# maxpit/human-pose-estimation

Hardware: AMD Instinct MI355X
Metric: images/sec (224x224, batch 256/GPU) (higher is better)
Workload: dtype f32; 1 GPU; batch=256/GPU 224x224x3 synthetic images, fp32 ResNet-50 v1 + 3-iter regressor + SMPL LBS at all 3 stages (configs[1] at batch 256; the BASELINE metric batch); global_batch=256, parallelism=dp1 (batch shard, replicated weights), regressor=synthetic 'survey' variant, input=float32 images resident in HBM

## Files before the change

human-pose-estimation_amd/csrc/bf16_rows.h:

```cpp
#pragma once
#include <hip/hip_runtime.h>

#include "hpe_internal.h"

#define BKE 64
#define RF 32

#define HPE_WAIT_VMCNT(n) __builtin_amdgcn_s_waitcnt(0x0F70 | ((n) & 15) | (((n) >> 4) << 14))
#define HPE_WAIT_LGKM0() __builtin_amdgcn_s_waitcnt(0xC07F)
```

human-pose-estimation_amd/csrc/conv_chain_f32.hip:

```cpp
#include <hip/hip_runtime.h>
#include <stdint.h>

#include "hpe_internal.h"

typedef float f32x16 __attribute__((ext_vector_type(16)));
typedef float f32x4 __attribute__((ext_vector_type(4)));
typedef const __attribute__((address_space(4))) float* cfloat_p;
typedef const __attribute__((address_space(4))) f32x4* cf32x4_p;

namespace {

__device__ __forceinline__ void dma16(const void* src, void* lds_dst) {
    __builtin_amdgcn_global_load_lds((const __attribute__((address_space(1))) void*)src, (__attribute__((address_space(3))) void*)lds_dst, 16, 0, 0);
}
__device__ __forceinline__ void dma16_nt(const void* src, void* lds_dst) {
    __builtin_amdgcn_global_load_lds((const __attribute__((address_space(1))) void*)src, (__attribute__((address_space(3))) void*)lds_dst, 16, 0, 2);
}
__device__ __forceinline__ void lds_barrier() { asm volatile("s_waitcnt lgkmcnt(0)\n\ts_barrier" ::: "memory"); }
__device__ __forceinline__ void wait_dma_leaving(int n, bool exact_counts) {
    if (!exact_counts) n = 0;
    switch (n) {
        case 4: asm volatile("s_waitcnt vmcnt(4)" ::: "memory"); break;
        case 8: asm volatile("s_waitcnt vmcnt(8)" ::: "memory"); break;
        default: asm volatile("s_waitcnt vmcnt(0)" ::: "memory"); break;
    }
}

template <int C, int CP>
__global__ __launch_bounds__(256, 2) void chain_expand_reduce_f32_kernel(ChainArgsF32 p) {
    constexpr int BM = 64, NC = 64, C4 = 4 * C;
    constexpr int KSA = C / 32, KSB = NC / 32, NCH = C4 / NC;
    constexpr int SLAB = BM * 128;
    constexpr int QBYTES = KSB * SLAB, QBUFS = 32768 / QBYTES;
    constexpr int WA_SLAB = NC * 128, WB_SLAB = CP * 128;
    constexpr int AT_OFF = 0, Q_OFF = KSA * SLAB, WA_OFF = Q_OFF + QBUFS * QBYTES, WB_OFF = WA_OFF + KSA * WA_SLAB;
    constexpr int LDS_BYTES = WB_OFF + KSB * WB_SLAB;
    constexpr int RI = KSB * 2, WIB = KSB * CP / 32, ST = NC / 16;
    static_assert(C == 64 && CP == 64, "stage 2 only: one 32-channel block per wave in both GEMMs");
    static_assert(QBUFS == 2 && NCH == 4 && LDS_BYTES <= 80 * 1024, "geometry");
    static_assert(RI == 4 && WIB == 4 && ST == 4, "the counted waits below know 0 / 4 / 8 only");

    __shared__ __attribute__((aligned(16))) unsigned char lds[LDS_BYTES];

// ... 48 lines not shown
#pragma unroll
        for (int s = 0; s < KSB; ++s) {
            const char* base = WBb + (c * NC + s * 32) * 4;
#pragma unroll
            for (int i = 0; i < CP / 32; ++i)
                dma16(base + (size_t)(32 * i) * p.ldw2a * 4 + off_wb, lds + WB_OFF + s * WB_SLAB + (wave + 4 * i) * 1024);
        }
    };

    const int wm = wave >> 1, wn = wave & 1;
    const int ar = wm * 32 + (lane & 31);
    const int a_off = ar * 128, a_x = (ar >> 1) & 7;
    const int wr = wn * 32 + (lane & 31);
    const int w_off = wr * 128, w_x = (wr >> 1) & 7;

    f32x16 accB;
#pragma unroll
    for (int e = 0; e < 16; ++e) accB[e] = 0.f;

    issue_at();
    issue_res(0);
    issue_wa(0);
    issue_wb(0);
    issue_res(1);

#pragma unroll
    for (int c = 0; c < NCH; ++c) {
        const int qb = c % QBUFS;
        wait_dma_leaving(c == 0 ? WIB + (QBUFS - 1) * RI : ST, full_tile);
        lds_barrier();
        if (c > 0) issue_wb(c);
        if (c > 0 && c - 1 + QBUFS < NCH) issue_res(c - 1 + QBUFS);

        f32x16 accA;
#pragma unroll
        for (int e = 0; e < 16; ++e) accA[e] = 0.f;
#pragma unroll
        for (int sa = 0; sa < KSA; ++sa)
#pragma unroll
            for (int g = 0; g < 4; ++g) {
                const int lc = 2 * g + hi;
                const f32x4 fa = *reinterpret_cast<const f32x4*>(lds + AT_OFF + sa * SLAB + a_off + ((lc ^ a_x) << 4));
                const f32x4 fw = *reinterpret_cast<const f32x4*>(lds + WA_OFF + sa * WA_SLAB + w_off + ((lc ^ w_x) << 4));
#pragma unroll
                for (int ks = 0; ks < 4; ++ks) accA = __builtin_amdgcn_mfma_f32_32x32x2f32(fw[ks], fa[ks], accA, 0, 0, 0);
            }

        {
            unsigned char* Qs = lds + Q_OFF + qb * QBYTES + wn * SLAB + a_off;
            cfloat_p scp = (cfloat_p)(p.scaleA + c * NC + wn * 32);
            cfloat_p shp = (cfloat_p)(p.shiftA + c * NC + wn * 32);
#pragma unroll
            for (int q = 0; q < 4; ++q) {
                unsigned char* qp = Qs + (((2 * q + hi) ^ a_x) << 4);
                const f32x4 rv = *reinterpret_cast<const f32x4*>(qp);
                const f32x4 sc_lo = *reinterpret_cast<cf32x4_p>(scp + 8 * q), sc_hi = *reinterpret_cast<cf32x4_p>(scp + 8 * q + 4);
                const f32x4 sh_lo = *reinterpret_cast<cf32x4_p>(shp + 8 * q), sh_hi = *reinterpret_cast<cf32x4_p>(shp + 8 * q + 4);
                f32x4 o;
#pragma unroll
                for (int k = 0; k < 4; ++k) {
                    const float sc = hi ? sc_hi[k] : sc_lo[k];
// ... 10 lines not shown
        {
            const unsigned char* Q = lds + Q_OFF + qb * QBYTES;
            constexpr int UPR = NC / 4;
#pragma unroll
            for (int pass = 0; pass < (BM * UPR) / 256; ++pass) {
                const int idx = pass * 256 + t;
                const int r = idx / UPR, u = idx - r * UPR;
                const f32x4 v = *reinterpret_cast<const f32x4*>(Q + (u >> 3) * SLAB + r * 128 + (((u & 7) ^ ((r >> 1) & 7)) << 4));
                const int m = m0 + r;
                if (m < p.M) __builtin_nontemporal_store(v, reinterpret_cast<f32x4*>(p.t3 + (size_t)m * C4 + c * NC + u * 4));
            }
        }
#pragma unroll
        for (int sb = 0; sb < KSB; ++sb) {
            const unsigned char* Q = lds + Q_OFF + qb * QBYTES + sb * SLAB;
#pragma unroll
            for (int g = 0; g < 4; ++g) {
                const int lc = 2 * g + hi;
                const f32x4 fa = *reinterpret_cast<const f32x4*>(Q + a_off + ((lc ^ a_x) << 4));
                const f32x4 fw = *reinterpret_cast<const f32x4*>(lds + WB_OFF + sb * WB_SLAB + w_off + ((lc ^ w_x) << 4));
#pragma unroll
                for (int ks = 0; ks < 4; ++ks) accB = __builtin_amdgcn_mfma_f32_32x32x2f32(fw[ks], fa[ks], accB, 0, 0, 0);
            }
        }
    }

    {
        unsigned char* Us = lds + AT_OFF + wn * SLAB + a_off;
        cfloat_p scp = (cfloat_p)(p.scaleB + wn * 32);
        cfloat_p shp = (cfloat_p)(p.shiftB + wn * 32);
#pragma unroll
        for (int q = 0; q < 4; ++q) {
            const f32x4 sc_lo = *reinterpret_cast<cf32x4_p>(scp + 8 * q), sc_hi = *reinterpret_cast<cf32x4_p>(scp + 8 * q + 4);
            const f32x4 sh_lo = *reinterpret_cast<cf32x4_p>(shp + 8 * q), sh_hi = *reinterpret_cast<cf32x4_p>(shp + 8 * q + 4);
            f32x4 o;
#pragma unroll
            for (int k = 0; k < 4; ++k) {
                const float sc = hi ? sc_hi[k] : sc_lo[k];
                const float sh = hi ? sh_hi[k] : sh_lo[k];
                o[k] = fmaxf(accB[4 * q + k] * sc + sh, 0.f);
            }
// ... 21 lines not shown
                else *reinterpret_cast<f32x4*>(p.u1 + (size_t)m * CP + u * 4) = v;
            }
        }
    }
}

}

bool hpe_chain_f32_supported(int C, int C4, int CP) { return C == 64 && C4 == 256 && CP == 64; }

hipError_t hpe_launch_chain_f32(const ChainArgsF32& p, int C, int C4, int CP, hipStream_t st) {
    if (!hpe_chain_f32_supported(C, C4, CP)) return hipErrorInvalidValue;
    if (p.M <= 0 || !p.t2 || !p.res || !p.w2c || !p.w2a || !p.t3 || !p.u1 || !p.scaleA || !p.shiftA || !p.scaleB || !p.shiftB) return hipErrorInvalidValue;
    if (p.ldw2c < C || p.ldw2a < C4 || (p.ldw2c % 4) != 0 || (p.ldw2a % 4) != 0) return hipErrorInvalidValue;
    if ((((uintptr_t)p.t2 | (uintptr_t)p.res | (uintptr_t)p.w2c | (uintptr_t)p.w2a | (uintptr_t)p.t3 | (uintptr_t)p.u1) & 15) != 0) return hipErrorInvalidValue;
    hipLaunchKernelGGL((chain_expand_reduce_f32_kernel<64, 64>), dim3((p.M + 63) / 64), dim3(256), 0, st, p);
    return hipGetLastError();
}

hipError_t hpe_chain_f32_occupancy(int* out) {
    return hipOccupancyMaxActiveBlocksPerMultiprocessor(out, reinterpret_cast<const void*>(chain_expand_reduce_f32_kernel<64, 64>), 256, 0);
}
```

human-pose-estimation_amd/csrc/conv_gemm.hip:

```cpp
#include <hip/hip_runtime.h>
#include <stdint.h>

#include "conv_gemm_common.h"
#include "gemm_contract.h"
#include "hpe_internal.h"

namespace {

template <int MODE, int BM, int BN, int WM, int WN>
__global__ __launch_bounds__(64 * WM * WN, (WM * WN) / 2) void conv_gemm_f32_dma_kernel(GemmArgs p) {
    constexpr int MT = BM / WM / 32;
    constexpr int NT = BN / WN / 32;
    constexpr int NW = WM * WN;
    constexpr int NTHR = 64 * NW;
    constexpr int AP = BM / (8 * NW);
    constexpr int BP = BN / (8 * NW);
    constexpr int EP = BN + 4;
    constexpr int BUF = (BM + BN) * BK;
    constexpr int LDS_FLOATS = (2 * BUF > BM * EP) ? 2 * BUF : BM * EP;
    static_assert(NW == 4 || NW == 8, "4 or 8 waves per workgroup");
    static_assert(AP >= 1 && BP >= 1, "tile too small for the wave count");

    __shared__ __attribute__((aligned(16))) float lds[LDS_FLOATS];

    const int total = p.n_mtiles * p.n_ntiles;
    const int bid = blockIdx.x;
    int tile, ks0 = 0, ks1 = p.K / BK, part = -1;
    if (p.split_k > 1) {
        tile = bid / p.split_k;
        part = bid - tile * p.split_k;
        const int S = p.K / BK;
        ks0 = (int)((long)part * S / p.split_k);
        ks1 = (int)((long)(part + 1) * S / p.split_k);
    } else {
        tile = xcd_remap(bid, total);
    }
// ... 36 lines not shown
#pragma unroll
    for (int j = 0; j < NT; ++j) {
        const int r = (wn * NT + j) * 32 + (lane & 31);
        b_row[j] = (BM + r) * BK;
        b_x[j] = (r >> 1) & 7;
    }
    const int hi = lane >> 5;

    f32x16 acc[MT][NT];
#pragma unroll
    for (int i = 0; i < MT; ++i)
#pragma unroll
        for (int j = 0; j < NT; ++j)
#pragma unroll
            for (int e = 0; e < 16; ++e) acc[i][j][e] = 0.f;

    constexpr int R_TPR = BN / 4, R_RPP = NTHR / R_TPR, R_NPASS = BM / R_RPP;
    constexpr bool R_PRE = (NW == 8) && R_NPASS <= 4;
    f32x4 rpre[R_PRE ? R_NPASS : 1];
    bool r_pre = false;
    if constexpr (R_PRE) {
        const int rr_ = t / R_TPR;
        const int n = n0 + (t - rr_ * R_TPR) * 4;
        r_pre = p.res != nullptr && p.res_prefetch && part < 0 && (n + 3) < p.N;
        if (r_pre) {
#pragma unroll
            for (int pass = 0; pass < R_NPASS; ++pass) {
                const int m = m0 + pass * R_RPP + rr_;
                rpre[pass] = HPE_RES_LOAD(reinterpret_cast<const f32x4*>(p.res + (size_t)(m < p.M ? m : p.M - 1) * p.ldres + n));
            }
        }
    }

    SlabPos sp = slab_seek<MODE>(p, ks0);

    auto issue_dma = [&](int slab, int buf) {
// ... 17 lines not shown
                                             (__attribute__((address_space(3))) void*)(lds + buf + (BM + (NW * i + wave) * 8) * BK), 16, 0,
                                             0);
        }
    };

    issue_dma(ks0, 0);
    __builtin_amdgcn_s_waitcnt(0x0F70);
    __syncthreads();

    for (int s = ks0; s < ks1; ++s) {
        const int cur = ((s - ks0) & 1) * BUF;
        if (s + 1 < ks1) {
            slab_advance<MODE>(p, sp);
            issue_dma(s + 1, BUF - cur);
        }
#pragma unroll
        for (int g = 0; g < 4; ++g) {
            f32x4 fa[MT], fb[NT];
            const int lc = 2 * g + hi;
#pragma unroll
            for (int i = 0; i < MT; ++i) fa[i] = *reinterpret_cast<const f32x4*>(&lds[cur + a_row[i] + ((lc ^ a_x[i]) << 2)]);
#pragma unroll
            for (int j = 0; j < NT; ++j) fb[j] = *reinterpret_cast<const f32x4*>(&lds[cur + b_row[j] + ((lc ^ b_x[j]) << 2)]);
#pragma unroll
            for (int ks = 0; ks < 4; ++ks)
#pragma unroll
                for (int i = 0; i < MT; ++i)
#pragma unroll
                    for (int j = 0; j < NT; ++j)
                        acc[i][j] = __builtin_amdgcn_mfma_f32_32x32x2f32(fa[i][ks], fb[j][ks], acc[i][j], 0, 0, 0);
        }
        __builtin_amdgcn_s_waitcnt(0x0F70);
        __syncthreads();
    }

    if (part >= 0) {
        f32x4* dst = reinterpret_cast<f32x4*>(p.partial) + (size_t)(tile * p.split_k + part) * (MT * NT * 4 * NTHR) + t;
#pragma unroll
        for (int i = 0; i < MT; ++i)
#pragma unroll
            for (int j = 0; j < NT; ++j)
#pragma unroll
                for (int qd = 0; qd < 4; ++qd) {
                    f32x4 v = {acc[i][j][4 * qd], acc[i][j][4 * qd + 1], acc[i][j][4 * qd + 2], acc[i][j][4 * qd + 3]};
                    dst[((i * NT + j) * 4 + qd) * NTHR] = v;
                }
        return;
    }
// ... 39 lines not shown
    }
    const f32x4 no_pre[1] = {{0.f, 0.f, 0.f, 0.f}};
    conv_epilogue<BM, BN, WM, WN>(p, lds, acc, mtile * BM, ntile * BN, t, lane, wm, wn, no_pre, false);
}

template <int MODE, int TILE>
hipError_t launch_cfg(GemmArgs& p, int splitk_min_slabs, hipStream_t st) {
    constexpr TileShape T = tile_shape(GEMM_K_F32, TILE);
    constexpr int BM = T.bm, BN = T.bn, WM = T.wm, WN = T.wn;
    p.n_mtiles = (p.M + BM - 1) / BM;
    p.n_ntiles = (p.N + BN - 1) / BN;
    const int grid = p.n_mtiles * p.n_ntiles;
    p.split_k = 1;
    if constexpr (WM * WN == 8) {
        p.res_prefetch = 1;
        hipLaunchKernelGGL((conv_gemm_f32_dma_kernel<MODE, BM, BN, WM, WN>), dim3(grid), dim3(512), 0, st, p);
        return hipGetLastError();
    } else {
        const int S = p.K / BK;
        if (p.partial && grid < 128 && S >= 2 * splitk_min_slabs) {
            int sk = 256 / grid;
            if (sk > S / splitk_min_slabs) sk = S / splitk_min_slabs;
            if (sk > 16) sk = 16;
            while (sk > 1 && (size_t)grid * sk * BM * BN > p.partial_floats) --sk;
            if (sk > 1) p.split_k = sk;
        }
        hipLaunchKernelGGL((conv_gemm_f32_dma_kernel<MODE, BM, BN, WM, WN>), dim3(grid * p.split_k), dim3(256), 0, st, p);
        hipError_t e = hipGetLastError();
        if (e != hipSuccess || p.split_k == 1) return e;
        hipLaunchKernelGGL((conv_gemm_fixup_kernel<BM, BN, WM, WN>), dim3(grid), dim3(256), 0, st, p);
        return hipGetLastError();
    }
}

template <int MODE>
hipError_t launch_mode(GemmArgs& p, int tile, int splitk_min_slabs, hipStream_t st) {
    switch (tile) {
        case TILE_128x128: return launch_cfg<MODE, TILE_128x128>(p, splitk_min_slabs, st);
        case TILE_128x64: return launch_cfg<MODE, TILE_128x64>(p, splitk_min_slabs, st);
        case TILE_64x64: return launch_cfg<MODE, TILE_64x64>(p, splitk_min_slabs, st);
        case TILE_64x128: return launch_cfg<MODE, TILE_64x128>(p, splitk_min_slabs, st);
        case TILE_128x128_W8: return launch_cfg<MODE, TILE_128x128_W8>(p, splitk_min_slabs, st);
// ... 24 lines not shown
```

human-pose-estimation_amd/csrc/conv_gemm_f32s.hip:

```cpp
#include <hip/hip_runtime.h>
#include <stdint.h>
#include <stdlib.h>

#include "conv_gemm_common.h"
#include "gemm_contract.h"
#include "hpe_internal.h"

namespace {

typedef __bf16 bf16x8 __attribute__((ext_vector_type(8)));

__device__ __forceinline__ void split3(const f32x4& lo, const f32x4& hi, bf16x8& h0, bf16x8& h1, bf16x8& h2) {
#pragma unroll
    for (int e = 0; e < 8; ++e) {
        const float x = e < 4 ? lo[e] : hi[e - 4];
        const __bf16 b0 = (__bf16)x;
        const float r1 = x - (float)b0;
        const __bf16 b1 = (__bf16)r1;
        const float r2 = r1 - (float)b1;
        h0[e] = b0;
        h1[e] = b1;
        h2[e] = (__bf16)r2;
    }
}

template <int MODE, int BM, int BN, int WM, int WN>
__global__ __launch_bounds__(64 * WM * WN, 2) void conv_gemm_f32s_dma_kernel(GemmArgs p) {
    constexpr int MT = BM / WM / 32;
    constexpr int NT = BN / WN / 32;
    constexpr int NW = WM * WN;
    constexpr int NTHR = 64 * NW;
    constexpr int AP = BM / (8 * NW);
    constexpr int BP = BN / (16 * NW);
    constexpr int A_BYTES = BM * BK * 4;
    constexpr int W_BYTES = BN * BK * 2;
    constexpr int BUF = A_BYTES + 3 * W_BYTES;
    constexpr int EPB = BM * (BN + 4) * 4;
    constexpr int LDS_BYTES = (2 * BUF > EPB) ? 2 * BUF : EPB;
    static_assert(NW == 4 || NW == 8, "4 or 8 waves per workgroup");
// ... 180 lines not shown
```

human-pose-estimation_amd/csrc/hpe_ctx.h:

```cpp
#pragma once
#include <hip/hip_runtime.h>

#include <cmath>
#include <cstdint>
#include <cstring>
#include <string>
#include <vector>

#include "../../include/hpe.h"
#include "hpe_internal.h"
#include "hpe_plan.h"

int fail(int code, const std::string& msg);

#define HIP_TRY(expr)                                                                                             \
    do {                                                                                                          \
        hipError_t _e = (expr);                                                                                   \
        if (_e != hipSuccess)                                                                                     \
            return fail(HPE_ERR_HIP, std::string(#expr) + ": " + hipGetErrorString(_e) + " (" __FILE__ ":" +      \
                                         std::to_string(__LINE__) + ")");                                         \
    } while (0)

struct ConvSpec {
    char name[24];
// ... 241 lines not shown
        if (_e != hipSuccess) return _e;         \
    } while (0)

enum { NEED_ENC = 1, NEED_REG = 2, NEED_SMPL = 4 };
int check_ready(hpe_ctx* c, int B, int need);

int finalize_impl(hpe_ctx* c);
void release_device_state(hpe_ctx* c);
int repack_encoder(hpe_ctx* c);

hipError_t run_conv(hpe_ctx* c, int idx, const ConvRoute& r, const float* x, int B, const float* res, int relu, float* y, hipStream_t st,
                    float* wino_v = nullptr, int slot = 0, const float* scale = nullptr, const float* shift = nullptr);
hipError_t run_conv_nhwc(hpe_ctx* c, int idx, const float* x, int B, const float* res, int relu, float* y, hipStream_t st,
                         const float* scale = nullptr, const float* shift = nullptr);
hipError_t run_chain(hpe_ctx* c, int i2c, bool first, const float* t2, const float* res, int B, float* t3, float* u1, hipStream_t st,
                     bool u1_slab8 = false);
hipError_t encoder_impl(hpe_ctx* c, const float* images, int B, float* features, int ldfeat, hipStream_t st);
hipError_t run_dense(hpe_ctx* c, const float* x, int lda, int M, int K, const float* w, int w_rows, int N, const float* scale, const float* shift,
                     const float* res, int ldres, int relu, float* y, int ldy, hipStream_t st, float* partial = nullptr, size_t partial_floats = 0);
hipError_t regress_impl(hpe_ctx* c, const float* th_prev, float* th_next, int B, hipStream_t st);
hipError_t features_proj(hpe_ctx* c, const float* features, int B, hipStream_t st);
hipError_t tail_impl(hpe_ctx* c, const float* feat, int B, const HpeOutputs* stage_outs, int n_outs, hipStream_t ts, hipEvent_t feat_free);
hipError_t join_tail(hpe_ctx* c, hipStream_t st);
int forward_impl(hpe_ctx* c, const float* images, int B, const HpeOutputs* stage_outs, int n_outs, hipStream_t st, bool pipelined);

size_t encoder_repack_reserve_floats();
int encoder_repack_reserve(hpe_ctx* c);
hipError_t encoder_repack_launch(hpe_ctx* c, const float* flat_dev, hipStream_t st);

hipError_t encoder_repack_stats_launch(hpe_ctx* c, hipStream_t st);

// ... 17 lines not shown
```

human-pose-estimation_amd/csrc/hpe_encoder.hip:

```cpp
#include <hip/hip_runtime.h>

#include <cmath>
#include <cstdint>
#include <cstdio>
#include <cstdlib>
#include <cstring>
#include <string>
#include <vector>

#include "hpe_ctx.h"

static hipError_t launch_gemm(hpe_ctx* c, GemmArgs& p, const ConvRoute& r, const void* w_split, hipStream_t st) {
    if (!r.concurrent) p.partial = c->partial, p.partial_floats = c->partial_floats;
    if (r.kernel == CONV_K_BF16 || r.kernel == CONV_K_BF16_P8) return hpe_launch_gemm_bf16(p, r.mode, r.tile, st);
    if (r.kernel != CONV_K_F32S) return hpe_launch_gemm(p, r.mode, r.tile, c->plan.splitk_min_slabs, st);
    if (!w_split) return hipErrorInvalidValue;
    p.w = static_cast<const float*>(w_split);
    p.w_piece = p.ldw;
    p.ldw *= 3;
    return hpe_launch_gemm_f32s(p, r.mode, r.tile, st);
}

hipError_t run_conv(hpe_ctx* c, int idx, const ConvRoute& r, const float* x, int B, const float* res, int relu, float* y, hipStream_t st,
                    float* wino_v, int slot, const float* scale, const float* shift) {
    const ConvSpec& s = specs()[idx];
    const ConvLayer& L = c->conv[idx];
    if (!scale) scale = L.scale;
    if (!shift) shift = L.shift;
    const int H = s.hin;
    const bool f2 = r.kernel == CONV_K_WINO || r.kernel == CONV_K_WINO_FUSED, f4 = r.kernel == CONV_K_WINO4 || r.kernel == CONV_K_WINO4_FUSED;
// ... 50 lines not shown

static hipError_t run_dual(hpe_ctx* c, int i2c, int i1, const ConvRoute& r, const float* t2, const float* x, int B, float* y, hipStream_t st) {
    const ConvSpec& s2 = specs()[i2c];
    const ConvSpec& s1 = specs()[i1];
    const ConvLayer& L = c->conv[i2c];
    GemmArgs p{};
    p.x = t2, p.x2 = x, p.w = L.w_dual, p.scale = c->ones, p.shift = L.shift_dual, p.y = y, p.zero = c->zeros;
    p.M = B * s2.hout * s2.hout, p.N = s2.cout, p.K = L.k_dual;
    p.k1_slabs = L.k1_dual / (c->bf16 ? 64 : 32), p.relu = 1;
    p.lda = s2.cin, p.ldw = L.k_dual, p.w_rows = round_up(s2.cout, 128), p.ldy = s2.cout;
    p.Hi = p.Wi = s1.hin, p.Cin = s1.cin, p.Ho = p.Wo = s1.hout, p.stride = s1.stride;
    return launch_gemm(c, p, r, L.w_dual_split, st);
}

hipError_t run_chain(hpe_ctx* c, int i2c, bool first, const float* t2, const float* res, int B, float* t3, float* u1, hipStream_t st,
                     bool u1_slab8) {
    const ConvSpec& s2 = specs()[i2c];
    const int inext = i2c + (first ? 2 : 1);
    const ConvSpec& sn = specs()[inext];
    const ConvLayer& L2 = c->conv[i2c];
    const ConvLayer& Ln = c->conv[inext];
    if (!c->bf16) {
        ChainArgsF32 q{};
        q.t2 = t2;
        q.res = res;
        q.w2c = L2.w;
        q.w2a = Ln.w;
        q.scaleA = L2.scale;
        q.shiftA = L2.shift;
        q.scaleB = Ln.scale;
        q.shiftB = Ln.shift;
        q.t3 = t3;
        q.u1 = u1;
        q.M = B * s2.hout * s2.hout;
        q.ldw2c = L2.k_pad;
        q.ldw2a = Ln.k_pad;
        q.u1_slab8 = u1_slab8 ? 1 : 0;
        return hpe_launch_chain_f32(q, s2.cin, s2.cout, sn.cout, st);
    }
    ChainArgs p{};
    p.t2 = reinterpret_cast<const __bf16*>(t2);
    if (first) {
        p.x2 = reinterpret_cast<const __bf16*>(res);
        p.w2c = reinterpret_cast<const __bf16*>(L2.w_dual);
        p.scaleA = c->ones;
        p.shiftA = L2.shift_dual;
        p.ldw2c = L2.k_dual;
    } else {
        p.res = reinterpret_cast<const __bf16*>(res);
        p.w2c = reinterpret_cast<const __bf16*>(L2.w);
        p.scaleA = L2.scale;
        p.shiftA = L2.shift;
// ... 82 lines not shown
        const BlockRoute br = route_block(c->plan, c->bf16, blk, q);
        if (have_2a) {
            if (c->timing >= 2) {
                HIPE(hipEventRecord(c->cev0[i2a], st));
                HIPE(hipEventRecord(c->cev1[i2a], st));
            }
        } else {
            HIPE(timed_conv(c, i2a, br.r2a, cur, B, nullptr, 1, T1, st));
        }
        have_2a = false;
        HIPE(timed_conv(c, i2b, br.r2b, T1, B, nullptr, 1, T2, st, wv, slot));
        const float* res = cur;
        if (br.join == JOIN_CHAIN) {
            const bool t2 = c->timing >= 2;
            if (t2) HIPE(hipEventRecord(c->cev0[i2c], st));
            HIPE(run_chain(c, i2c, first, T2, cur, B, nxt, T1, st, br.u1_slab8));
            if (t2) {
                HIPE(hipEventRecord(c->cev1[i2c], st));
                if (first) {
                    HIPE(hipEventRecord(c->cev0[i1], st));
                    HIPE(hipEventRecord(c->cev1[i1], st));
                }
            }
            have_2a = true;
        } else if (br.join == JOIN_DUAL) {
            const bool t2 = c->timing >= 2;
            if (t2) HIPE(hipEventRecord(c->cev0[i2c], st));
            HIPE(run_dual(c, i2c, i1, br.r2c, T2, cur, B, nxt, st));
            if (t2) {
                HIPE(hipEventRecord(c->cev1[i2c], st));
                HIPE(hipEventRecord(c->cev0[i1], st));
// ... 143 lines not shown
```

human-pose-estimation_amd/csrc/hpe_internal.h:

```cpp
#pragma once
#include <hip/hip_runtime.h>
#include <stddef.h>

#include "../../include/hpe.h"

typedef float f32x4 __attribute__((ext_vector_type(4)));
typedef float f32x16 __attribute__((ext_vector_type(16)));

template <typename Id>
__device__ __forceinline__ int xcd_remap(Id bid, int total) {
    const int xcd = bid & 7;
    const int q = total >> 3, rr = total & 7;
    return (xcd < rr ? xcd * (q + 1) : rr * (q + 1) + (xcd - rr) * q) + (bid >> 3);
}

inline dim3 grid1(long n) { return dim3((unsigned)((n + 255) / 256)); }

enum GemmMode { GEMM_DENSE = 0, GEMM_STRIDED = 1, GEMM_CONV3 = 2, GEMM_STEM = 3, GEMM_DUAL = 4 };
enum GemmTile { TILE_128x128 = 0, TILE_128x64 = 1, TILE_64x64 = 2, TILE_64x128 = 3, TILE_128x128_W8 = 4, TILE_128x64_W8 = 5, TILE_256x128_W8 = 6,
                TILE_P8_256x256 = 7  };

struct GemmArgs {
    const float* x;
    const float* w;
// ... 4 lines not shown
    int M, N, K;
    int lda, ldw, ldy, ldres, w_rows;
    int relu;
    int Hi, Wi, Cin, Ho, Wo, stride, cin_slabs;
    int n_mtiles, n_ntiles;
    int split_k;
    float* partial;
    size_t partial_floats;
    const float* zero;
    void* reserved;
    const float* x2;
    int k1_slabs;
    int res_prefetch;
    int y_slab8;
    int w_piece;
};

hipError_t hpe_launch_gemm(GemmArgs p, int mode, int tile, int splitk_min_slabs, hipStream_t st, int* split_k_out = nullptr);
hipError_t hpe_launch_gemm_f32s(GemmArgs p, int mode, int tile, hipStream_t st);

size_t hpe_wino_v_floats(int B, int H, int W, int C);
hipError_t hpe_wino_init_device();
#define HPE_WINO_WS_FLOATS 65536
struct WinoStreamK {
    float* ws;
    unsigned* flags;
    unsigned epoch;
    int n_wg;
    unsigned* err;
};
// ... 38 lines not shown
    __bf16* y;
    int M, N, ldw, relu;
    int n_ntiles;
    int two;
};
bool hpe_halo3_bf16_supported(int HW, int Cin, int N);
hipError_t hpe_launch_halo3_bf16(const Halo3Args& p, int HW, int Cin, hipStream_t st);

bool hpe_chain_bf16_supported(int C, int C4, int CP, int C2);
hipError_t hpe_launch_chain_bf16(const ChainArgs& p, int C, int C4, int CP, int C2, hipStream_t st);
hipError_t hpe_chain_bf16_occupancy(int out[3]);
struct ChainArgsF32 {
    const float *t2, *res, *w2c, *w2a, *scaleA, *shiftA, *scaleB, *shiftB;
    float *t3, *u1;
    int M, ldw2c, ldw2a, u1_slab8;
};
bool hpe_chain_f32_supported(int C, int C4, int CP);
hipError_t hpe_launch_chain_f32(const ChainArgsF32& p, int C, int C4, int CP, hipStream_t st);
hipError_t hpe_chain_f32_occupancy(int* out);
hipError_t hpe_launch_f32_to_bf16(const float* x, void* y, long n, hipStream_t st);
hipError_t hpe_launch_bf16_to_f32(const void* x, float* y, long n, hipStream_t st);
hipError_t hpe_launch_pad_input_bf16(const float* img, void* out, int B, int H, int W, int Hp, int Wp, hipStream_t st);
hipError_t hpe_launch_maxpool_bf16(const void* x, void* y, int B, int H, int C, hipStream_t st);
hipError_t hpe_launch_avgpool_bf16(const void* x, float* y, int B, int HW, int C, int ldy, hipStream_t st);

hipError_t hpe_launch_stem_fused(const float* img, const void* w, const float* scale, const float* shift, void* y, int B, int R, int bf16,
                                 hipStream_t st);
hipError_t hpe_stem_fused_init_device();
int hpe_stem_fused_pick_rows(int B);

// ... 143 lines not shown
```

human-pose-estimation_amd/csrc/hpe_plan.h:

```cpp
#pragma once
#include "../../include/hpe.h"
#include "hpe_internal.h"

struct HpePlan {
    int n_streams = 2;
    int dual_gemm = 1;
    int stem_fused = 1;
    int wino_min_c = 128;
    int wino_min_items = 128;
    int wino_fused = 1;
    int wino_fused_min_hw = 28;
    int mesh_a2b = 0;
    int wino_f4 = 7;
    int wino4_fused = 0;
    int bf16_p8 = 0;
    int wino4_ksplit = 1;
    int chain_fuse = 0;
    int halo3 = 0;
    int f32_split = 0;
    int chunk_images = 0;
    int min_chunk = 32;
    int halo3_two = 4;
    int f32s_min_tiles = 128;
    int wino_streamk = 0;
    int concurrent_tiles = 0;
    int bf16_w8_min_tiles = 128;
    int wide128_min_tiles = 384;
    int force_wide = -1;
    int splitk_min_slabs = 4;
    int wino4_min_items = 64;
    int wino4_n32 = 256;
    int w4_abl = 0;
};

constexpr int PLAN_BF16_128_MIN_TILES = 192;
constexpr int PLAN_BF16_P8_MIN_N = 256;
constexpr int PLAN_BF16_P8_MIN_K = 512;
constexpr int PLAN_EXPAND_SMALL_GRID = 128;
constexpr int PLAN_SHORTK_TILE = TILE_128x64_W8;
constexpr int PLAN_F32S_TILE = TILE_128x128;
constexpr int PLAN_F32S_EXPAND_TILE = TILE_128x128_W8;
constexpr int PLAN_F32S_EXPAND_MIN_K = 256;

HpePlan hpe_resolve_plan(const HpeConfig& cfg);

inline int stage_bit(int hout) { return hout >= 56 ? 1 : (hout >= 28 ? 2 : (hout >= 14 ? 4 : 8)); }
// ... 25 lines not shown
```

human-pose-estimation_amd/csrc/hpe_plan.hip:

```cpp
#include <hip/hip_runtime.h>

#include <climits>
#include <cmath>
#include <cstdint>
#include <cstdio>
#include <cstdlib>
#include <cstring>
#include <string>
#include <vector>

#include "gemm_contract.h"
#include "hpe_ctx.h"

namespace {

struct Network {
    std::vector<ConvSpec> specs;
    std::vector<ResBlock> blocks;
};

Network build_network() {
    Network net;
    std::vector<ConvSpec>& v = net.specs;
    auto add = [&](const std::string& n, const std::string& b, int kh, int cin, int cout, int s, int hin, int hout) {
// ... 72 lines not shown
    {&HpePlan::chain_fuse, &HpeConfig::chain_fuse, "HPE_CHAIN", {8, 7}, {8, 23}, NO_LO, NO_HI},
    {&HpePlan::halo3, &HpeConfig::halo3, "HPE_HALO3", {15, 15}, {0, 15}, NO_LO, NO_HI},
    {&HpePlan::f32_split, &HpeConfig::f32_split, "HPE_F32_SPLIT", {14, 14}, {15, 0}, NO_LO, NO_HI},
    {&HpePlan::chunk_images, nullptr, "HPE_CHUNK", {0, 0}, {ANY, ANY}, NO_LO, NO_HI},
    {&HpePlan::min_chunk, nullptr, "HPE_MIN_CHUNK", {32, 24}, {ANY, ANY}, NO_LO, NO_HI},
    {&HpePlan::halo3_two, nullptr, "HPE_HALO3_TWO", {4, 4}, {7, 7}, NO_LO, NO_HI},
    {&HpePlan::f32s_min_tiles, nullptr, "HPE_F32S_MIN_TILES", {128, 128}, {ANY, ANY}, NO_LO, NO_HI},
    {&HpePlan::wino_streamk, nullptr, "HPE_WINO_STREAMK", {0, 0}, {ANY, ANY}, NO_LO, NO_HI},
    {&HpePlan::concurrent_tiles, nullptr, "HPE_CONCURRENT_TILES", {0, 0}, {ANY, ANY}, NO_LO, NO_HI},
    {&HpePlan::bf16_w8_min_tiles, nullptr, "HPE_BF16_W8_MIN_TILES", {128, 128}, {ANY, ANY}, NO_LO, NO_HI},
    {&HpePlan::wide128_min_tiles, nullptr, "HPE_WIDE128_MIN_TILES", {384, 384}, {ANY, ANY}, NO_LO, NO_HI},
    {&HpePlan::force_wide, nullptr, "HPE_TILE_WIDE", {-1, -1}, {ANY, ANY}, NO_LO, NO_HI},
    {&HpePlan::splitk_min_slabs, nullptr, "HPE_SPLITK_SLABS", {4, 4}, {ANY, ANY}, 2, NO_HI},
    {&HpePlan::wino4_min_items, nullptr, "HPE_WINO4_MIN_ITEMS", {64, 64}, {ANY, ANY}, NO_LO, NO_HI},
    {&HpePlan::wino4_n32, nullptr, "HPE_WINO4_N32", {256, 256}, {ANY, ANY}, NO_LO, NO_HI},
    {&HpePlan::w4_abl, nullptr, "HPE_W4_ABL", {0, 0}, {ANY, ANY}, NO_LO, NO_HI},
};

HpePlan hpe_resolve_plan(const HpeConfig& cfg) {
    const int dt = cfg.encoder_dtype == 1 ? 1 : 0;
    HpePlan pl;
    for (const PlanOption& o : kPlanOptions) {
        int v = o.dflt[dt];
        const char* e = getenv(o.env);
        if (o.cfg && cfg.*o.cfg >= 0) v = cfg.*o.cfg;
        else if (e && o.member == &HpePlan::mesh_a2b) v = e[0] == 'v' ? 1 : (e[0] == 'm' ? 2 : 0);
        else if (e) v = atoi(e);
        v &= o.mask[dt];
        pl.*o.member = v < o.lo ? o.lo : (v > o.hi ? o.hi : v);
    }
// ... 130 lines not shown
```

human-pose-estimation_amd/engine.py:

```python
from __future__ import annotations

import ctypes as C

import numpy as np

from . import _lib
from .critic_spec import PARAM_FLOATS
from .regressor_spec import PARAM_FLOATS as REGRESSOR_PARAM_FLOATS
from .resnet_spec import CONV_SPECS, ENCODER_PARAM_FLOATS, ENCODER_STAT_FLOATS

NUM_VERTS = _lib.NUM_VERTS


def _torch():
    import torch

    return torch


def _require_cuda_tensor(t, name, shape_tail=None):
    torch = _torch()
    if not isinstance(t, torch.Tensor):
        raise TypeError("%s must be a torch.Tensor on the GPU" % name)
    if not t.is_cuda:
# ... 791 lines not shown
        images = _require_cuda_tensor(images, "images", (224, 224, 3))
        y = self._new(images.shape[0], 56, 56, 64)
        _lib.check(self.lib.hpe_debug_stem(self._h, images.data_ptr(), images.shape[0], int(rows_per_strip), y.data_ptr(), self._stream()))
        return y

    def joint_regress(self, X, use_kp_regressor=True):
        X = _require_cuda_tensor(X, "X", (NUM_VERTS, 3))
        K = self.num_kp if use_kp_regressor else 24
        out = self._new(X.shape[0], K, 3)
        _lib.check(self.lib.hpe_debug_joint_regress(self._h, X.data_ptr(), X.shape[0], int(use_kp_regressor), out.data_ptr(), self._stream()))
        return out

    def encoder_kernel_description(self):
        if self.encoder_dtype == "fp32":
            return ("conv_gemm_f32s_dma_kernel (the 1x1 / strided / dual-source layers of stages 3-5 on the bf16 matrix cores, operands split "
                    "exactly into three bf16 pieces) + conv_gemm_f32_dma_kernel (the other 1x1 layers) + w4_input_kernel + w4_gemm_kernel / w4_gemm32_kernel "
                    "(the 13 3x3 layers on the 28x28 / 14x14 / 7x7 maps as fp32 Winograd F(4x4,3x3); F(2x2,3x3) / direct below 64 work "
                    "items) + wino_fused_kernel (the three 56x56 3x3 layers, F(2x2,3x3)) + stem_fused_f32s_kernel (image and weights split like the 1x1 layers) -- the 53 conv layers of one "
                    "step, priced at their direct-convolution FLOPs")
        return ("conv_gemm_bf16_dma_kernel (1x1 / strided / dual-source layers) + chain_expand_reduce_bf16_kernel (branch2c + next branch2a of "
                "stages 2-3 as one launch) + conv3_halo_bf16_kernel (the sixteen 3x3 layers, tile + halo resident in LDS) + stem_fused_bf16_kernel "
                "-- the 53 conv layers of one step, priced at their algorithmic HBM bytes")

    def enable_timing(self, level=1):
        _lib.check(self.lib.hpe_enable_timing(self._h, int(level)))

    def timings(self):
        ms = (C.c_float * 5)()
        _lib.check(self.lib.hpe_get_timings(self._h, ms))
        return dict(encoder_ms=ms[0], conv_ms=ms[1], regress_smpl_ms=ms[2], total_ms=ms[4])

# ... 70 lines not shown
```

Before: 21940 images/sec.

## Split fp32 operands into three bf16 pieces for dense GEMM and chain kernels

```diff
diff --git a/human-pose-estimation_amd/csrc/bf16_rows.h b/human-pose-estimation_amd/csrc/bf16_rows.h
--- a/human-pose-estimation_amd/csrc/bf16_rows.h
+++ b/human-pose-estimation_amd/csrc/bf16_rows.h
@@ -8,3 +8,42 @@
 
 #define HPE_WAIT_VMCNT(n) __builtin_amdgcn_s_waitcnt(0x0F70 | ((n) & 15) | (((n) >> 4) << 14))
 #define HPE_WAIT_LGKM0() __builtin_amdgcn_s_waitcnt(0xC07F)
+
+typedef __bf16 bf16x8 __attribute__((ext_vector_type(8)));
+
+__device__ __forceinline__ void split3(const f32x4& lo, const f32x4& hi, bf16x8& h0, bf16x8& h1, bf16x8& h2) {
+#pragma unroll
+    for (int e = 0; e < 8; ++e) {
+        const float x = e < 4 ? lo[e] : hi[e - 4];
+        const __bf16 b0 = (__bf16)x;
+        const float r1 = x - (float)b0;
+        const __bf16 b1 = (__bf16)r1;
+        const float r2 = r1 - (float)b1;
+        h0[e] = b0;
+        h1[e] = b1;
+        h2[e] = (__bf16)r2;
+    }
+}
+
+typedef float f32x2 __attribute__((ext_vector_type(2)));
+typedef __bf16 bf16x2 __attribute__((ext_vector_type(2)));
+typedef unsigned u32x2 __attribute__((ext_vector_type(2)));
+__device__ __forceinline__ f32x2 bf16x2_widen(bf16x2 h) {
+    const unsigned u = __builtin_bit_cast(unsigned, h);
+    const u32x2 w = {u << 16, u & 0xffff0000u};
+    return __builtin_bit_cast(f32x2, w);
+}
+__device__ __forceinline__ void split3_pk(const f32x4& lo, const f32x4& hi, bf16x8& h0, bf16x8& h1, bf16x8& h2) {
+#pragma unroll
+    for (int e = 0; e < 4; ++e) {
+        const f32x2 x = e < 2 ? f32x2{lo[2 * e], lo[2 * e + 1]} : f32x2{hi[2 * e - 4], hi[2 * e - 3]};
+        const bf16x2 b0 = __builtin_convertvector(x, bf16x2);
+        const f32x2 r1 = x - bf16x2_widen(b0);
+        const bf16x2 b1 = __builtin_convertvector(r1, bf16x2);
+        const f32x2 r2 = r1 - bf16x2_widen(b1);
+        const bf16x2 b2 = __builtin_convertvector(r2, bf16x2);
+        h0[2 * e] = b0[0], h0[2 * e + 1] = b0[1];
+        h1[2 * e] = b1[0], h1[2 * e + 1] = b1[1];
+        h2[2 * e] = b2[0], h2[2 * e + 1] = b2[1];
+    }
+}
diff --git a/human-pose-estimation_amd/csrc/conv_chain_f32.hip b/human-pose-estimation_amd/csrc/conv_chain_f32.hip
--- a/human-pose-estimation_amd/csrc/conv_chain_f32.hip
+++ b/human-pose-estimation_amd/csrc/conv_chain_f32.hip
@@ -1,6 +1,7 @@
 #include <hip/hip_runtime.h>
 #include <stdint.h>
 
+#include "bf16_rows.h"
 #include "hpe_internal.h"
 
 typedef float f32x16 __attribute__((ext_vector_type(16)));
@@ -26,7 +27,18 @@
     }
 }
 
-template <int C, int CP>
+enum { CORE_F32 = 0, CORE_SPLIT = 1 };
+
+__device__ __forceinline__ void mfma_split6(const bf16x8 (&w)[3], const bf16x8 (&a)[3], f32x16& acc, f32x16& acx) {
+    acx = __builtin_amdgcn_mfma_f32_32x32x16_bf16(w[0], a[2], acx, 0, 0, 0);
+    acx = __builtin_amdgcn_mfma_f32_32x32x16_bf16(w[1], a[1], acx, 0, 0, 0);
+    acx = __builtin_amdgcn_mfma_f32_32x32x16_bf16(w[2], a[0], acx, 0, 0, 0);
+    acx = __builtin_amdgcn_mfma_f32_32x32x16_bf16(w[0], a[1], acx, 0, 0, 0);
+    acx = __builtin_amdgcn_mfma_f32_32x32x16_bf16(w[1], a[0], acx, 0, 0, 0);
+    acc = __builtin_amdgcn_mfma_f32_32x32x16_bf16(w[0], a[0], acc, 0, 0, 0);
+}
+
+template <int C, int CP, int CORE>
 __global__ __launch_bounds__(256, 2) void chain_expand_reduce_f32_kernel(ChainArgsF32 p) {
     constexpr int BM = 64, NC = 64, C4 = 4 * C;
     constexpr int KSA = C / 32, KSB = NC / 32, NCH = C4 / NC;
@@ -105,9 +117,14 @@
     const int wr = wn * 32 + (lane & 31);
     const int w_off = wr * 128, w_x = (wr >> 1) & 7;
 
-    f32x16 accB;
-#pragma unroll
-    for (int e = 0; e < 16; ++e) accB[e] = 0.f;
+    f32x16 accB, accBx;
+#pragma unroll
+    for (int e = 0; e < 16; ++e) accB[e] = accBx[e] = 0.f;
+    bf16x8 at[CORE == CORE_SPLIT ? 2 * KSA : 1][3];
+    auto frag3 = [&](const unsigned char* row, int x, int q, bf16x8 (&h)[3]) {
+        const int lc = 4 * q + 2 * hi;
+        split3_pk(*reinterpret_cast<const f32x4*>(row + ((lc ^ x) << 4)), *reinterpret_cast<const f32x4*>(row + (((lc + 1) ^ x) << 4)), h[0], h[1], h[2]);
+    };
 
     issue_at();
     issue_res(0);
@@ -126,16 +143,32 @@
         f32x16 accA;
 #pragma unroll
         for (int e = 0; e < 16; ++e) accA[e] = 0.f;
-#pragma unroll
-        for (int sa = 0; sa < KSA; ++sa)
-#pragma unroll
-            for (int g = 0; g < 4; ++g) {
-                const int lc = 2 * g + hi;
-                const f32x4 fa = *reinterpret_cast<const f32x4*>(lds + AT_OFF + sa * SLAB + a_off + ((lc ^ a_x) << 4));
-                const f32x4 fw = *reinterpret_cast<const f32x4*>(lds + WA_OFF + sa * WA_SLAB + w_off + ((lc ^ w_x) << 4));
-#pragma unroll
-                for (int ks = 0; ks < 4; ++ks) accA = __builtin_amdgcn_mfma_f32_32x32x2f32(fw[ks], fa[ks], accA, 0, 0, 0);
-            }
+        if constexpr (CORE == CORE_SPLIT) {
+            f32x16 accAx;
+#pragma unroll
+            for (int e = 0; e < 16; ++e) accAx[e] = 0.f;
+#pragma unroll
+            for (int sa = 0; sa < KSA; ++sa)
+#pragma unroll
+                for (int q = 0; q < 2; ++q) {
+                    if (c == 0) frag3(lds + AT_OFF + sa * SLAB + a_off, a_x, q, at[2 * sa + q]);
+                    bf16x8 w[3];
+                    frag3(lds + WA_OFF + sa * WA_SLAB + w_off, w_x, q, w);
+                    mfma_split6(w, at[2 * sa + q], accA, accAx);
+                }
+            accA += accAx;
+        } else {
+#pragma unroll
+            for (int sa = 0; sa < KSA; ++sa)
+#pragma unroll
+                for (int g = 0; g < 4; ++g) {
+                    const int lc = 2 * g + hi;
+                    const f32x4 fa = *reinterpret_cast<const f32x4*>(lds + AT_OFF + sa * SLAB + a_off + ((lc ^ a_x) << 4));
+                    const f32x4 fw = *reinterpret_cast<const f32x4*>(lds + WA_OFF + sa * WA_SLAB + w_off + ((lc ^ w_x) << 4));
+#pragma unroll
+                    for (int ks = 0; ks < 4; ++ks) accA = __builtin_amdgcn_mfma_f32_32x32x2f32(fw[ks], fa[ks], accA, 0, 0, 0);
+                }
+        }
 
         {
             unsigned char* Qs = lds + Q_OFF + qb * QBYTES + wn * SLAB + a_off;
@@ -176,17 +209,28 @@
 #pragma unroll
         for (int sb = 0; sb < KSB; ++sb) {
             const unsigned char* Q = lds + Q_OFF + qb * QBYTES + sb * SLAB;
-#pragma unroll
-            for (int g = 0; g < 4; ++g) {
-                const int lc = 2 * g + hi;
-                const f32x4 fa = *reinterpret_cast<const f32x4*>(Q + a_off + ((lc ^ a_x) << 4));
-                const f32x4 fw = *reinterpret_cast<const f32x4*>(lds + WB_OFF + sb * WB_SLAB + w_off + ((lc ^ w_x) << 4));
-#pragma unroll
-                for (int ks = 0; ks < 4; ++ks) accB = __builtin_amdgcn_mfma_f32_32x32x2f32(fw[ks], fa[ks], accB, 0, 0, 0);
-            }
-        }
-    }
-
+            if constexpr (CORE == CORE_SPLIT) {
+#pragma unroll
+                for (int q = 0; q < 2; ++q) {
+                    bf16x8 a[3], w[3];
+                    frag3(Q + a_off, a_x, q, a);
+                    frag3(lds + WB_OFF + sb * WB_SLAB + w_off, w_x, q, w);
+                    mfma_split6(w, a, accB, accBx);
+                }
+            } else {
+#pragma unroll
+                for (int g = 0; g < 4; ++g) {
+                    const int lc = 2 * g + hi;
+                    const f32x4 fa = *reinterpret_cast<const f32x4*>(Q + a_off + ((lc ^ a_x) << 4));
+                    const f32x4 fw = *reinterpret_cast<const f32x4*>(lds + WB_OFF + sb * WB_SLAB + w_off + ((lc ^ w_x) << 4));
+#pragma unroll
+                    for (int ks = 0; ks < 4; ++ks) accB = __builtin_amdgcn_mfma_f32_32x32x2f32(fw[ks], fa[ks], accB, 0, 0, 0);
+                }
+            }
+        }
+    }
+
+    if constexpr (CORE == CORE_SPLIT) accB += accBx;
     {
         unsigned char* Us = lds + AT_OFF + wn * SLAB + a_off;
         cfloat_p scp = (cfloat_p)(p.scaleB + wn * 32);
@@ -238,10 +282,11 @@
     if (p.M <= 0 || !p.t2 || !p.res || !p.w2c || !p.w2a || !p.t3 || !p.u1 || !p.scaleA || !p.shiftA || !p.scaleB || !p.shiftB) return hipErrorInvalidValue;
     if (p.ldw2c < C || p.ldw2a < C4 || (p.ldw2c % 4) != 0 || (p.ldw2a % 4) != 0) return hipErrorInvalidValue;
     if ((((uintptr_t)p.t2 | (uintptr_t)p.res | (uintptr_t)p.w2c | (uintptr_t)p.w2a | (uintptr_t)p.t3 | (uintptr_t)p.u1) & 15) != 0) return hipErrorInvalidValue;
-    hipLaunchKernelGGL((chain_expand_reduce_f32_kernel<64, 64>), dim3((p.M + 63) / 64), dim3(256), 0, st, p);
+    if (p.core_split) hipLaunchKernelGGL((chain_expand_reduce_f32_kernel<64, 64, CORE_SPLIT>), dim3((p.M + 63) / 64), dim3(256), 0, st, p);
+    else hipLaunchKernelGGL((chain_expand_reduce_f32_kernel<64, 64, CORE_F32>), dim3((p.M + 63) / 64), dim3(256), 0, st, p);
     return hipGetLastError();
 }
 
 hipError_t hpe_chain_f32_occupancy(int* out) {
-    return hipOccupancyMaxActiveBlocksPerMultiprocessor(out, reinterpret_cast<const void*>(chain_expand_reduce_f32_kernel<64, 64>), 256, 0);
-}
+    return hipOccupancyMaxActiveBlocksPerMultiprocessor(out, reinterpret_cast<const void*>(chain_expand_reduce_f32_kernel<64, 64, CORE_F32>), 256, 0);
+}
diff --git a/human-pose-estimation_amd/csrc/conv_gemm.hip b/human-pose-estimation_amd/csrc/conv_gemm.hip
--- a/human-pose-estimation_amd/csrc/conv_gemm.hip
+++ b/human-pose-estimation_amd/csrc/conv_gemm.hip
@@ -1,14 +1,17 @@
 #include <hip/hip_runtime.h>
 #include <stdint.h>
 
+#include "bf16_rows.h"
 #include "conv_gemm_common.h"
 #include "gemm_contract.h"
 #include "hpe_internal.h"
 
 namespace {
 
-template <int MODE, int BM, int BN, int WM, int WN>
-__global__ __launch_bounds__(64 * WM * WN, (WM * WN) / 2) void conv_gemm_f32_dma_kernel(GemmArgs p) {
+enum { CORE_F32 = 0, CORE_SPLIT = 1 };
+
+template <int MODE, int BM, int BN, int WM, int WN, int CORE>
+__global__ __launch_bounds__(64 * WM * WN, CORE == CORE_SPLIT ? 6 : (WM * WN) / 2) void conv_gemm_f32_dma_kernel(GemmArgs p) {
     constexpr int MT = BM / WM / 32;
     constexpr int NT = BN / WN / 32;
     constexpr int NW = WM * WN;
@@ -20,6 +23,8 @@
     constexpr int LDS_FLOATS = (2 * BUF > BM * EP) ? 2 * BUF : BM * EP;
     static_assert(NW == 4 || NW == 8, "4 or 8 waves per workgroup");
     static_assert(AP >= 1 && BP >= 1, "tile too small for the wave count");
+    static_assert(CORE == CORE_F32 || (MT == 1 && NT == 1 && NW == 8 && (MODE == GEMM_DENSE || MODE == GEMM_DUAL)),
+                  "split core: one 32 x 32 block per wave, 8 waves, dense / dual-source only");
 
     __shared__ __attribute__((aligned(16))) float lds[LDS_FLOATS];
 
@@ -86,12 +91,17 @@
         for (int j = 0; j < NT; ++j)
 #pragma unroll
             for (int e = 0; e < 16; ++e) acc[i][j][e] = 0.f;
+    f32x16 acx;
+    if constexpr (CORE == CORE_SPLIT) {
+#pragma unroll
+        for (int e = 0; e < 16; ++e) acx[e] = 0.f;
+    }
 
     constexpr int R_TPR = BN / 4, R_RPP = NTHR / R_TPR, R_NPASS = BM / R_RPP;
     constexpr bool R_PRE = (NW == 8) && R_NPASS <= 4;
     f32x4 rpre[R_PRE ? R_NPASS : 1];
     bool r_pre = false;
-    if constexpr (R_PRE) {
+    if constexpr (R_PRE && CORE == CORE_F32) {
         const int rr_ = t / R_TPR;
         const int n = n0 + (t - rr_ * R_TPR) * 4;
         r_pre = p.res != nullptr && p.res_prefetch && part < 0 && (n + 3) < p.N;
@@ -139,24 +149,57 @@
             slab_advance<MODE>(p, sp);
             issue_dma(s + 1, BUF - cur);
         }
-#pragma unroll
-        for (int g = 0; g < 4; ++g) {
-            f32x4 fa[MT], fb[NT];
-            const int lc = 2 * g + hi;
-#pragma unroll
-            for (int i = 0; i < MT; ++i) fa[i] = *reinterpret_cast<const f32x4*>(&lds[cur + a_row[i] + ((lc ^ a_x[i]) << 2)]);
-#pragma unroll
-            for (int j = 0; j < NT; ++j) fb[j] = *reinterpret_cast<const f32x4*>(&lds[cur + b_row[j] + ((lc ^ b_x[j]) << 2)]);
-#pragma unroll
-            for (int ks = 0; ks < 4; ++ks)
-#pragma unroll
-                for (int i = 0; i < MT; ++i)
-#pragma unroll
-                    for (int j = 0; j < NT; ++j)
-                        acc[i][j] = __builtin_amdgcn_mfma_f32_32x32x2f32(fa[i][ks], fb[j][ks], acc[i][j], 0, 0, 0);
+        if constexpr (CORE == CORE_SPLIT) {
+#pragma unroll
+            for (int q = 0; q < 2; ++q) {
+                const int lc = 4 * q + 2 * hi;
+                const f32x4 a_lo = *reinterpret_cast<const f32x4*>(&lds[cur + a_row[0] + ((lc ^ a_x[0]) << 2)]);
+                const f32x4 a_up = *reinterpret_cast<const f32x4*>(&lds[cur + a_row[0] + (((lc + 1) ^ a_x[0]) << 2)]);
+                const f32x4 w_lo = *reinterpret_cast<const f32x4*>(&lds[cur + b_row[0] + ((lc ^ b_x[0]) << 2)]);
+                const f32x4 w_up = *reinterpret_cast<const f32x4*>(&lds[cur + b_row[0] + (((lc + 1) ^ b_x[0]) << 2)]);
+                bf16x8 a0, a1, a2, w0, w1, w2;
+                split3_pk(a_lo, a_up, a0, a1, a2);
+                split3_pk(w_lo, w_up, w0, w1, w2);
+                acx = __builtin_amdgcn_mfma_f32_32x32x16_bf16(a2, w0, acx, 0, 0, 0);
+                acx = __builtin_amdgcn_mfma_f32_32x32x16_bf16(a1, w1, acx, 0, 0, 0);
+                acx = __builtin_amdgcn_mfma_f32_32x32x16_bf16(a0, w2, acx, 0, 0, 0);
+                acx = __builtin_amdgcn_mfma_f32_32x32x16_bf16(a1, w0, acx, 0, 0, 0);
+                acx = __builtin_amdgcn_mfma_f32_32x32x16_bf16(a0, w1, acx, 0, 0, 0);
+                acc[0][0] = __builtin_amdgcn_mfma_f32_32x32x16_bf16(a0, w0, acc[0][0], 0, 0, 0);
+            }
+        } else {
+#pragma unroll
+            for (int g = 0; g < 4; ++g) {
+                f32x4 fa[MT], fb[NT];
+                const int lc = 2 * g + hi;
+#pragma unroll
+                for (int i = 0; i < MT; ++i) fa[i] = *reinterpret_cast<const f32x4*>(&lds[cur + a_row[i] + ((lc ^ a_x[i]) << 2)]);
+#pragma unroll
+                for (int j = 0; j < NT; ++j) fb[j] = *reinterpret_cast<const f32x4*>(&lds[cur + b_row[j] + ((lc ^ b_x[j]) << 2)]);
+#pragma unroll
+                for (int ks = 0; ks < 4; ++ks)
+#pragma unroll
+                    for (int i = 0; i < MT; ++i)
+#pragma unroll
+                        for (int j = 0; j < NT; ++j)
+                            acc[i][j] = __builtin_amdgcn_mfma_f32_32x32x2f32(fa[i][ks], fb[j][ks], acc[i][j], 0, 0, 0);
+            }
         }
         __builtin_amdgcn_s_waitcnt(0x0F70);
         __syncthreads();
+    }
+    if constexpr (CORE == CORE_SPLIT) {
+        acc[0][0] += acx;
+        const int rr_ = t / R_TPR;
+        const int n = n0 + (t - rr_ * R_TPR) * 4;
+        r_pre = p.res != nullptr && p.res_prefetch && (n + 3) < p.N;
+        if (r_pre) {
+#pragma unroll
+            for (int pass = 0; pass < R_NPASS; ++pass) {
+                const int m = m0 + pass * R_RPP + rr_;
+                rpre[pass] = HPE_RES_LOAD(reinterpret_cast<const f32x4*>(p.res + (size_t)(m < p.M ? m : p.M - 1) * p.ldres + n));
+            }
+        }
     }
 
     if (part >= 0) {
@@ -226,7 +269,13 @@
     p.split_k = 1;
     if constexpr (WM * WN == 8) {
         p.res_prefetch = 1;
-        hipLaunchKernelGGL((conv_gemm_f32_dma_kernel<MODE, BM, BN, WM, WN>), dim3(grid), dim3(512), 0, st, p);
+        if constexpr (TILE == TILE_128x64_W8 && (MODE == GEMM_DENSE || MODE == GEMM_DUAL)) {
+            if (p.core_split) {
+                hipLaunchKernelGGL((conv_gemm_f32_dma_kernel<MODE, BM, BN, WM, WN, CORE_SPLIT>), dim3(grid), dim3(512), 0, st, p);
+                return hipGetLastError();
+            }
+        }
+        hipLaunchKernelGGL((conv_gemm_f32_dma_kernel<MODE, BM, BN, WM, WN, CORE_F32>), dim3(grid), dim3(512), 0, st, p);
         return hipGetLastError();
     } else {
         const int S = p.K / BK;
@@ -237,7 +286,7 @@
             while (sk > 1 && (size_t)grid * sk * BM * BN > p.partial_floats) --sk;
             if (sk > 1) p.split_k = sk;
         }
-        hipLaunchKernelGGL((conv_gemm_f32_dma_kernel<MODE, BM, BN, WM, WN>), dim3(grid * p.split_k), dim3(256), 0, st, p);
+        hipLaunchKernelGGL((conv_gemm_f32_dma_kernel<MODE, BM, BN, WM, WN, CORE_F32>), dim3(grid * p.split_k), dim3(256), 0, st, p);
         hipError_t e = hipGetLastError();
         if (e != hipSuccess || p.split_k == 1) return e;
         hipLaunchKernelGGL((conv_gemm_fixup_kernel<BM, BN, WM, WN>), dim3(grid), dim3(256), 0, st, p);
diff --git a/human-pose-estimation_amd/csrc/conv_gemm_f32s.hip b/human-pose-estimation_amd/csrc/conv_gemm_f32s.hip
--- a/human-pose-estimation_amd/csrc/conv_gemm_f32s.hip
+++ b/human-pose-estimation_amd/csrc/conv_gemm_f32s.hip
@@ -2,27 +2,12 @@
 #include <stdint.h>
 #include <stdlib.h>
 
+#include "bf16_rows.h"
 #include "conv_gemm_common.h"
 #include "gemm_contract.h"
 #include "hpe_internal.h"
 
 namespace {
-
-typedef __bf16 bf16x8 __attribute__((ext_vector_type(8)));
-
-__device__ __forceinline__ void split3(const f32x4& lo, const f32x4& hi, bf16x8& h0, bf16x8& h1, bf16x8& h2) {
-#pragma unroll
-    for (int e = 0; e < 8; ++e) {
-        const float x = e < 4 ? lo[e] : hi[e - 4];
-        const __bf16 b0 = (__bf16)x;
-        const float r1 = x - (float)b0;
-        const __bf16 b1 = (__bf16)r1;
-        const float r2 = r1 - (float)b1;
-        h0[e] = b0;
-        h1[e] = b1;
-        h2[e] = (__bf16)r2;
-    }
-}
 
 template <int MODE, int BM, int BN, int WM, int WN>
 __global__ __launch_bounds__(64 * WM * WN, 2) void conv_gemm_f32s_dma_kernel(GemmArgs p) {
diff --git a/human-pose-estimation_amd/csrc/hpe_ctx.h b/human-pose-estimation_amd/csrc/hpe_ctx.h
--- a/human-pose-estimation_amd/csrc/hpe_ctx.h
+++ b/human-pose-estimation_amd/csrc/hpe_ctx.h
@@ -279,7 +279,7 @@
 hipError_t run_conv_nhwc(hpe_ctx* c, int idx, const float* x, int B, const float* res, int relu, float* y, hipStream_t st,
                          const float* scale = nullptr, const float* shift = nullptr);
 hipError_t run_chain(hpe_ctx* c, int i2c, bool first, const float* t2, const float* res, int B, float* t3, float* u1, hipStream_t st,
-                     bool u1_slab8 = false);
+                     bool u1_slab8 = false, bool concurrent = false);
 hipError_t encoder_impl(hpe_ctx* c, const float* images, int B, float* features, int ldfeat, hipStream_t st);
 hipError_t run_dense(hpe_ctx* c, const float* x, int lda, int M, int K, const float* w, int w_rows, int N, const float* scale, const float* shift,
                      const float* res, int ldres, int relu, float* y, int ldy, hipStream_t st, float* partial = nullptr, size_t partial_floats = 0);
diff --git a/human-pose-estimation_amd/csrc/hpe_encoder.hip b/human-pose-estimation_amd/csrc/hpe_encoder.hip
--- a/human-pose-estimation_amd/csrc/hpe_encoder.hip
+++ b/human-pose-estimation_amd/csrc/hpe_encoder.hip
@@ -13,7 +13,10 @@
 static hipError_t launch_gemm(hpe_ctx* c, GemmArgs& p, const ConvRoute& r, const void* w_split, hipStream_t st) {
     if (!r.concurrent) p.partial = c->partial, p.partial_floats = c->partial_floats;
     if (r.kernel == CONV_K_BF16 || r.kernel == CONV_K_BF16_P8) return hpe_launch_gemm_bf16(p, r.mode, r.tile, st);
-    if (r.kernel != CONV_K_F32S) return hpe_launch_gemm(p, r.mode, r.tile, c->plan.splitk_min_slabs, st);
+    if (r.kernel != CONV_K_F32S) {
+        p.core_split = !r.concurrent && (c->plan.f32_core_split & 1);
+        return hpe_launch_gemm(p, r.mode, r.tile, c->plan.splitk_min_slabs, st);
+    }
     if (!w_split) return hipErrorInvalidValue;
     p.w = static_cast<const float*>(w_split);
     p.w_piece = p.ldw;
@@ -94,7 +97,7 @@
 }
 
 hipError_t run_chain(hpe_ctx* c, int i2c, bool first, const float* t2, const float* res, int B, float* t3, float* u1, hipStream_t st,
-                     bool u1_slab8) {
+                     bool u1_slab8, bool concurrent) {
     const ConvSpec& s2 = specs()[i2c];
     const int inext = i2c + (first ? 2 : 1);
     const ConvSpec& sn = specs()[inext];
@@ -116,6 +119,7 @@
         q.ldw2c = L2.k_pad;
         q.ldw2a = Ln.k_pad;
         q.u1_slab8 = u1_slab8 ? 1 : 0;
+        q.core_split = !concurrent && (c->plan.f32_core_split & 2);
         return hpe_launch_chain_f32(q, s2.cin, s2.cout, sn.cout, st);
     }
     ChainArgs p{};
@@ -228,7 +232,7 @@
         if (br.join == JOIN_CHAIN) {
             const bool t2 = c->timing >= 2;
             if (t2) HIPE(hipEventRecord(c->cev0[i2c], st));
-            HIPE(run_chain(c, i2c, first, T2, cur, B, nxt, T1, st, br.u1_slab8));
+            HIPE(run_chain(c, i2c, first, T2, cur, B, nxt, T1, st, br.u1_slab8, concurrent));
             if (t2) {
                 HIPE(hipEventRecord(c->cev1[i2c], st));
                 if (first) {
diff --git a/human-pose-estimation_amd/csrc/hpe_internal.h b/human-pose-estimation_amd/csrc/hpe_internal.h
--- a/human-pose-estimation_amd/csrc/hpe_internal.h
+++ b/human-pose-estimation_amd/csrc/hpe_internal.h
@@ -42,6 +42,7 @@
     int res_prefetch;
     int y_slab8;
     int w_piece;
+    int core_split;
 };
 
 hipError_t hpe_launch_gemm(GemmArgs p, int mode, int tile, int splitk_min_slabs, hipStream_t st, int* split_k_out = nullptr);
@@ -110,6 +111,7 @@
     const float *t2, *res, *w2c, *w2a, *scaleA, *shiftA, *scaleB, *shiftB;
     float *t3, *u1;
     int M, ldw2c, ldw2a, u1_slab8;
+    int core_split;
 };
 bool hpe_chain_f32_supported(int C, int C4, int CP);
 hipError_t hpe_launch_chain_f32(const ChainArgsF32& p, int C, int C4, int CP, hipStream_t st);
diff --git a/human-pose-estimation_amd/csrc/hpe_plan.h b/human-pose-estimation_amd/csrc/hpe_plan.h
--- a/human-pose-estimation_amd/csrc/hpe_plan.h
+++ b/human-pose-estimation_amd/csrc/hpe_plan.h
@@ -30,6 +30,7 @@
     int splitk_min_slabs = 4;
     int wino4_min_items = 64;
     int wino4_n32 = 256;
+    int f32_core_split = 3;
     int w4_abl = 0;
 };
 
diff --git a/human-pose-estimation_amd/csrc/hpe_plan.hip b/human-pose-estimation_amd/csrc/hpe_plan.hip
--- a/human-pose-estimation_amd/csrc/hpe_plan.hip
+++ b/human-pose-estimation_amd/csrc/hpe_plan.hip
@@ -110,6 +110,7 @@
     {&HpePlan::splitk_min_slabs, nullptr, "HPE_SPLITK_SLABS", {4, 4}, {ANY, ANY}, 2, NO_HI},
     {&HpePlan::wino4_min_items, nullptr, "HPE_WINO4_MIN_ITEMS", {64, 64}, {ANY, ANY}, NO_LO, NO_HI},
     {&HpePlan::wino4_n32, nullptr, "HPE_WINO4_N32", {256, 256}, {ANY, ANY}, NO_LO, NO_HI},
+    {&HpePlan::f32_core_split, nullptr, "HPE_F32_CORE_SPLIT", {3, 0}, {3, 0}, NO_LO, NO_HI},
     {&HpePlan::w4_abl, nullptr, "HPE_W4_ABL", {0, 0}, {ANY, ANY}, NO_LO, NO_HI},
 };
 
diff --git a/human-pose-estimation_amd/engine.py b/human-pose-estimation_amd/engine.py
--- a/human-pose-estimation_amd/engine.py
+++ b/human-pose-estimation_amd/engine.py
@@ -829,7 +829,8 @@
     def encoder_kernel_description(self):
         if self.encoder_dtype == "fp32":
             return ("conv_gemm_f32s_dma_kernel (the 1x1 / strided / dual-source layers of stages 3-5 on the bf16 matrix cores, operands split "
-                    "exactly into three bf16 pieces) + conv_gemm_f32_dma_kernel (the other 1x1 layers) + w4_input_kernel + w4_gemm_kernel / w4_gemm32_kernel "
+                    "exactly into three bf16 pieces) + conv_gemm_f32_dma_kernel (the other 1x1 layers; fp32 MFMA in launches of concurrent batch chunks, else the "
+                    "eight-wave 128x64 tile and the chain kernel split both operands the same way in registers) + w4_input_kernel + w4_gemm_kernel / w4_gemm32_kernel "
                     "(the 13 3x3 layers on the 28x28 / 14x14 / 7x7 maps as fp32 Winograd F(4x4,3x3); F(2x2,3x3) / direct below 64 work "
                     "items) + wino_fused_kernel (the three 56x56 3x3 layers, F(2x2,3x3)) + stem_fused_f32s_kernel (image and weights split like the 1x1 layers) -- the 53 conv layers of one "
                     "step, priced at their direct-convolution FLOPs")
```

Measured after the change: 21930 images/sec. Within noise of the previous version (-0.0%).
